# redwarp/kmeans-gpu

Hardware: AMD Instinct MI355X
Metric: pixels/sec per Lloyd iteration (8192x8192, k=256) (higher is better)
Workload: dtype f32; 1 GPU; synthetic uniform RGBA 8192x8192 (seed 0x5EED0003), k=256, one Lloyd iteration = update + assign (labels written every iteration) + accumulate; width=8192, height=8192, k=256, collective_backend=none (one rank), collective_ranks=1, label_pass=before the next iteration, update=by the last launch of the assign pass (kmg_lloyd_assign_update)

## Files before the change

### kmeans-gpu_amd/csrc/kmg_cube.hip

```cpp

#include "kmg_internal.h"
#include "kmg_table_dev.h"

#include <hip/hip_fp16.h>
#include <stdlib.h>

namespace kmg {

typedef float f32x2 __attribute__((ext_vector_type(2)));


namespace {

constexpr uint32_t kMaxListed = 32;
constexpr uint32_t kMaxLong = 256;
constexpr uint32_t kLongFlag = 0x200u;

__device__ __forceinline__ uint32_t sel3(uint32_t i, uint32_t x0, uint32_t x1, uint32_t x2)
{
    return i == 0u ? x0 : (i == 1u ? x1 : x2);
}

__device__ __forceinline__ int round_dir(int g, int m)
{
    const int a = g < 0 ? -g : g;
    const int r = (4 * a >= 3 * m ? 1 : 0) + (4 * a >= m ? 1 : 0);
    return g < 0 ? -r : r;
}

typedef unsigned short u16x2 __attribute__((ext_vector_type(2)));

__device__ __forceinline__ uint32_t group8_or(uint32_t v)
{
    v |= dpp_u32<kDppXor1>(v);
    v |= dpp_u32<kDppXor2>(v);
    v |= dpp_u32<kDppHalfMirror>(v);
    return v;
}

__device__ __forceinline__ uint32_t group8_min_u32(uint32_t v)
{
    v = min(v, dpp_u32<kDppXor1>(v));
    v = min(v, dpp_u32<kDppXor2>(v));
    v = min(v, dpp_u32<kDppHalfMirror>(v));
    return v;
}

__device__ __forceinline__ uint32_t group8_max_u32(uint32_t v)
{
    v = max(v, dpp_u32<kDppXor1>(v));
    v = max(v, dpp_u32<kDppXor2>(v));
    v = max(v, dpp_u32<kDppHalfMirror>(v));
    return v;
}



__device__ __forceinline__ uint32_t cell_pair_entry(const uint32_t idx[8], uint32_t occ, uint32_t lane)
{
    uint32_t rem = occ;
    uint32_t lab0 = 0, lab1 = 0, lab2 = 0, cnt0 = 0, cnt1 = 0, cnt2 = 0, msk0 = 0, msk1 = 0, msk2 = 0, n_occ = 0;
#pragma unroll
    for (int t = 0; t < 3; ++t) {
        const unsigned long long any = __ballot(rem != 0u);
        if (any) {
            uint32_t mine = 0;
#pragma unroll
            for (int q = 7; q >= 0; --q) mine = ((rem >> q) & 1u) ? idx[q] : mine;
            const uint32_t v = lane_value(mine, (uint32_t)__builtin_ctzll(any));
            uint32_t mm = 0;
#pragma unroll
            for (int q = 0; q < 8; ++q) mm |= (idx[q] == v ? 1u : 0u) << q;
            mm &= rem;
            rem &= ~mm;
            const uint32_t packed = wave_add_u32((uint32_t)__builtin_popcount(mm) | (t == 0 ? (uint32_t)__builtin_popcount(occ) << 10 : 0u));
            const uint32_t c = packed & 1023u;
            if (t == 0) { lab0 = v; msk0 = mm; cnt0 = c; n_occ = packed >> 10; }
            if (t == 1) { lab1 = v; msk1 = mm; cnt1 = c; }
            if (t == 2) { lab2 = v; msk2 = mm; cnt2 = c; }
        }
    }
    uint32_t a = 0;
    if (cnt1 > cnt0) a = 1;
    if (cnt2 > sel3(a, cnt0, cnt1, cnt2)) a = 2;
    uint32_t b = a == 0u ? 1u : 0u;
    if (a != 1u && b != 1u && cnt1 > sel3(b, cnt0, cnt1, cnt2)) b = 1;
    if (a != 2u && cnt2 > sel3(b, cnt0, cnt1, cnt2)) b = 2;
    const uint32_t labA = sel3(a, lab0, lab1, lab2), labB = sel3(b, lab0, lab1, lab2);
    const uint32_t mA = sel3(a, msk0, msk1, msk2), mB = sel3(b, msk0, msk1, msk2);
    const uint32_t rest = occ & ~mA;
    const uint32_t nA = sel3(a, cnt0, cnt1, cnt2), nR = n_occ - nA;
    if (nR == 0u) return pair_entry(labA, labA, 0u, 0u, 0u);

    const uint32_t half = ((lane >> 5) & 1u) | (((lane >> 4) & 1u) << 10) | (((lane >> 3) & 1u) << 20);
    const uint32_t hR = wave_add_u32((uint32_t)__builtin_popcount(rest) * half);
    const uint32_t hA = wave_add_u32((uint32_t)__builtin_popcount(mA) * half);
    const int gx = (int)((hR & 1023u) * nA) - (int)((hA & 1023u) * nR);
    const int gy = (int)(((hR >> 10) & 1023u) * nA) - (int)(((hA >> 10) & 1023u) * nR);
    const int gz = (int)((hR >> 20) * nA) - (int)((hA >> 20) * nR);
    const int ax = gx < 0 ? -gx : gx, ay = gy < 0 ? -gy : gy, az = gz < 0 ? -gz : gz;
    const int m = ax > ay ? (ax > az ? ax : az) : (ay > az ? ay : az);
    int nx = 2, ny = 0, nz = 0;
    if (m > 0) { nx = round_dir(gx, m); ny = round_dir(gy, m); nz = round_dir(gz, m); }

    const int xl = (int)(((lane >> 5) & 1u) * 4u + ((lane >> 1) & 3u));
    const int yl = (int)(((lane >> 4) & 1u) * 4u + (lane & 1u) * 2u);
    const int zl = (int)(((lane >> 3) & 1u) * 4u);
    const int bias = 7 * ((nx < 0 ? -nx : 0) + (ny < 0 ? -ny : 0) + (nz < 0 ? -nz : 0));
    const int p0 = nx * xl + ny * yl + nz * zl + bias;
    int p[8];
#pragma unroll
    for (int q = 0; q < 8; ++q) p[q] = p0 + ny * (q >> 2) + nz * (q & 3);
    const uint32_t notB = occ & ~mB;
    uint32_t tl = 63u, hi = 64u;
#pragma unroll
    for (int q = 0; q < 8; ++q) {
        if ((rest >> q) & 1u) tl = min(tl, (uint32_t)p[q]);
        if ((notB >> q) & 1u) hi = min(hi, (uint32_t)(63 - p[q]));
    }
    u16x2 packed = __builtin_bit_cast(u16x2, tl | (hi << 16));
    packed = __builtin_elementwise_min(packed, __builtin_bit_cast(u16x2, dpp_u32<kDppXor1>(__builtin_bit_cast(uint32_t, packed))));
    packed = __builtin_elementwise_min(packed, __builtin_bit_cast(u16x2, dpp_u32<kDppXor2>(__builtin_bit_cast(uint32_t, packed))));
    packed = __builtin_elementwise_min(packed, __builtin_bit_cast(u16x2, dpp_u32<kDppHalfMirror>(__builtin_bit_cast(uint32_t, packed))));
    packed = __builtin_elementwise_min(packed, __builtin_bit_cast(u16x2, dpp_u32<kDppMirror>(__builtin_bit_cast(uint32_t, packed))));
    packed = __builtin_elementwise_min(packed, __builtin_bit_cast(u16x2, (uint32_t)__builtin_amdgcn_update_dpp(-1, (int)__builtin_bit_cast(uint32_t, packed), 0x142, 0xA, 0xF, false)));
    packed = __builtin_elementwise_min(packed, __builtin_bit_cast(u16x2, (uint32_t)__builtin_amdgcn_update_dpp(-1, (int)__builtin_bit_cast(uint32_t, packed), 0x143, 0xC, 0xF, false)));
    const uint32_t pk = lane_value(__builtin_bit_cast(uint32_t, packed), 63);
    const int tlo = (int)(pk & 0xFFFFu);
    const int thi = 63 - (int)(pk >> 16);
    const int w = thi + 1 > tlo ? thi + 1 - tlo : 0;
    const uint32_t code = pair_dir_code(nx, ny, nz);
    if (w <= 6) return pair_entry(labA, labB, code, (uint32_t)tlo, (uint32_t)w);
    uint32_t low = 0, high = 0;
#pragma unroll
    for (int q = 0; q < 8; ++q) {
        if ((occ >> q) & 1u) { low += p[q] < tlo ? 1u : 0u; high += p[q] > thi ? 1u : 0u; }
    }
    const uint32_t lh = wave_add_u32(low | (high << 10));
    if ((lh & 1023u) >= (lh >> 10)) return pair_entry(labA, labB, code, (uint32_t)tlo, 7u);
    const int range = 7 * ((nx < 0 ? -nx : nx) + (ny < 0 ? -ny : ny) + (nz < 0 ? -nz : nz));
    return pair_entry(labB, labA, pair_dir_code(-nx, -ny, -nz), (uint32_t)(range - thi), 7u);
}

__device__ __forceinline__ uint32_t merge_state(uint32_t a, uint32_t b)
{
    return (a == kSubEmpty) ? b : ((b == kSubEmpty || b == a) ? a : (uint32_t)kSubMixed);
}

template <typename LabelT>
__device__ __forceinline__ void store_labels64(LabelT *dst64, uint32_t label, uint32_t lane)
{
    if (sizeof(LabelT) == 1) {
        const uint32_t t = label | (dpp_u32<kDppXor1>(label) << 8);
        const uint32_t u = t | (dpp_u32<kDppXor2>(t) << 16);
        if ((lane & 3u) == 0u) reinterpret_cast<uint32_t *>(dst64)[lane >> 2] = u;
    } else {
        const uint32_t t = label | (dpp_u32<kDppXor1>(label) << 16);
        if ((lane & 1u) == 0u) reinterpret_cast<uint32_t *>(dst64)[lane >> 1] = t;
    }
}


struct alignas(16) CellWork {
    uint16_t list[kMaxListed];
    unsigned long long br[4];
    uint32_t npop;
    uint32_t scan_set;
    uint32_t pad[6];
};
static_assert(sizeof(CellWork) == 128, "CellWork layout");

constexpr uint32_t kPairPending = 0xFFFFFFFEu;

constexpr uint32_t kLongSegs = 16, kLongSegCap = kCells / kLongSegs, kLongCount = 0, kLongCells = 64;
constexpr size_t kListsWords = kLongCells + kCells;
constexpr uint32_t kItemCands = 12;

__device__ __forceinline__ void flush_bins(const unsigned long long *bins, uint32_t k, uint32_t repl, uint32_t bin_stride,
                                           int64_t *sums, uint32_t n_rows)
{
    __syncthreads();
    unsigned long long *row = reinterpret_cast<unsigned long long *>(sums) + (uint64_t)(blockIdx.x % n_rows) * 4ull * k;
    for (uint32_t i = threadIdx.x; i < 4u * k; i += blockDim.x) {
        unsigned long long v = 0ull;
        for (uint32_t r = 0; r < repl; ++r) v += bins[(uint64_t)r * bin_stride + i];
        if (v) atomicAdd(row + i, v);
    }
}

__device__ __forceinline__ uint2 long_list_stage(const float4 *s_cent, const unsigned long long *s_masks, uint16_t *s_long,
                                              unsigned long long *s_sub, float4 sb0, float4 sb1, float4 sb2, uint32_t npop,
                                              uint32_t words, uint64_t *sub_masks_cell)
{
    const uint32_t lane = threadIdx.x & 63u;
// ... 1423 lines not shown
            } else if (valid) {
                uint4 *dst = reinterpret_cast<uint4 *>(s_lbl + slot * kCellColours + sub * 64u);
                dst[0] = xv; dst[1] = xv; dst[2] = xv; dst[3] = xv;
            }
        }
        unsigned long long pend0_b = 0ull;
        {
            const uint32_t rank = (uint32_t)__builtin_popcount(scan8 & ((1u << sub) - 1u));
            const bool head = open && (rank & 1u) == 0u;
            const uint32_t after = scan8 & ~((2u << sub) - 1u);
            const uint32_t s1 = after ? (uint32_t)__builtin_ctz(after) : 8u;
            const uint32_t un = listed ? (nm | ((head && s1 < 8u) ? s_mask[threadIdx.x - sub + s1] : 0u)) : 0u;
            const uint32_t n_un = (uint32_t)__builtin_popcount(un);
            const uint32_t type = unlisted ? 2u : (n_un > kItemCands ? 1u : 0u);
            const bool pend = valid && !uniform && sub == 0u;
            if (pend) s_left[slot] = ((uint32_t)__builtin_popcount(scan8) + 1u) >> 1;
            pend0_b = __ballot(pend && scan8 == 0u);
            const unsigned long long item_b = __ballot(head);
            if (bal_state) {
                const uint32_t cost = wave_add_u32(head ? 4u + (type == 2u ? npop : n_un) : 0u);
                if (lane == 0u) bal_state[(bal_pass & 1u) * 2u * kOneTaskSlots + kOneTaskSlots + blockIdx.x * kOneWaves + wv] = (uint16_t)min(cost, 65535u);
            }
            uint32_t i_base = 0u;
            if (lane == 0u && item_b) i_base = atomicAdd(&s_count[0], (uint32_t)__builtin_popcountll(item_b));
            i_base = __builtin_amdgcn_readfirstlane(i_base);
            if (head) {
                uint32_t iw0 = un, iw1 = 0u, iw2 = 0u;
                if (type == 0u) {
                    iw0 = 0u;
                    uint32_t q = 0u;
                    for (uint32_t m = un; m; m &= m - 1u, ++q) {
                        const uint32_t cc = (uint32_t)s_list[slot * kMaxListed + (uint32_t)__builtin_ctz(m)] << (8u * (q & 3u));
                        iw0 |= q < 4u ? cc : 0u; iw1 |= (q >= 4u && q < 8u) ? cc : 0u; iw2 |= q >= 8u ? cc : 0u;
                    }
                }
                s_item[i_base + bits_below_lane(item_b)] = make_uint4(slot | (sub << 7) | (s1 << 10) | (n_un << 14) | (type << 30), iw0, iw1, iw2);
            }
            if (stats) {
                st_single += (uint32_t)__builtin_popcountll(__ballot(single && sub == 0u));
                st_multi += (uint32_t)__builtin_popcountll(__ballot(valid && !single && sub == 0u));
                st_unlisted += (uint32_t)__builtin_popcountll(__ballot(unlisted && sub == 0u));
                st_decided += (uint32_t)__builtin_popcountll(__ballot(was_decided));
                st_scanned += (uint32_t)__builtin_popcountll(__ballot(mine || (unlisted && occupied)));
                st_cands += wave_add_u32(mine ? np0 : ((unlisted && occupied) ? npop : 0u));
                st_removed += wave_add_u32((uint32_t)__builtin_popcount(sm & ~nm));
                st_one += (uint32_t)__builtin_popcountll(__ballot(one));
            }
        }
        KMG_STAMP(4);
        __syncthreads();
        const uint32_t n_items = s_count[0];
        KMG_STAMP_VALUE(8, n_items); KMG_STAMP_VALUE(10, s_count[8]);

        auto cell_entry = [&](const uint32_t ps) {
            const uint32_t pcell = __builtin_amdgcn_readfirstlane(s_cell[ps]);
            const uint2 lv = *reinterpret_cast<const uint2 *>(s_lbl + ps * kCellColours + lane * 8u);
            uint32_t e = kPairPending;
            if (!(flags & kCubeNoEntries)) {
                const uint32_t occ = (uint32_t)s_occ[ps * 64u + lane];
                uint32_t idx[8];
#pragma unroll
                for (uint32_t q = 0; q < 4u; ++q) { idx[q] = (lv.x >> (8u * q)) & 0xFFu; idx[4u + q] = (lv.y >> (8u * q)) & 0xFFu; }
                e = cell_pair_entry(idx, occ, lane);
            }
            if (lane == 0u) pair_entries[pcell] = e;
            *reinterpret_cast<uint2 *>(colour_labels + (uint64_t)pcell * kCellColours + lane * 8u) = lv;
        };

        {
            uint32_t A_h = 0u, A_w0 = 0u, A_w1 = 0u, A_w2 = 0u, B_h = 0u, B_w0 = 0u, B_w1 = 0u, B_w2 = 0u, C_h = 0u, C_w0 = 0u, C_w1 = 0u, C_w2 = 0u;
            float4 A_v0, A_v1, B_v0, B_v1, C_v0, C_v1;
            uint32_t A_c0 = 1u, A_c1 = 1u, B_c0 = 1u, B_c1 = 1u, C_c0 = 1u, C_c1 = 1u;
            long long A_g = 0, B_g = 0, C_g = 0;
            bool A_ok = false, B_ok = false, C_ok = false;
#define KMG_REQUEST_ITEM(X)                                                                                       \
            do {                                                                                                  \
                uint32_t next_ = 0u;                                                                              \
                if (lane == 0u) next_ = atomicAdd(&s_count[4], 1u);                                               \
                next_ = __builtin_amdgcn_readfirstlane(next_);                                                    \
                X##_ok = next_ < n_items;                                                                         \
                const uint4 it_ = s_item[next_ < n_items ? next_ : 0u];                                           \
                X##_h = __builtin_amdgcn_readfirstlane(it_.x); X##_w0 = __builtin_amdgcn_readfirstlane(it_.y);    \
                X##_w1 = __builtin_amdgcn_readfirstlane(it_.z); X##_w2 = __builtin_amdgcn_readfirstlane(it_.w);   \
                const uint32_t cell_ = __builtin_amdgcn_readfirstlane(s_cell[X##_h & 127u]);                       \
                const uint32_t c0_ = cell_ * kCellColours + ((X##_h >> 7) & 7u) * 64u + lane;                     \
                const uint32_t c1_ = cell_ * kCellColours + ((X##_h >> 10) & 7u) * 64u + lane;    \
                X##_v0 = lab_table[c0_]; X##_v1 = lab_table[c1_];                                                 \
                if (SUMS) { X##_c0 = hist[c0_]; X##_c1 = hist[c1_]; X##_g = sub_agg[(uint64_t)cell_ * 32u + (lane & 31u)]; } \
            } while (0)
            auto scan_item = [&](const uint32_t hdr, const uint32_t w0, const uint32_t w1, const uint32_t w2, const float4 v0, const float4 v1,
                                 const uint32_t cnt0, const uint32_t cnt1, const long long sagg) {
                const uint32_t islot = hdr & 127u, s0 = (hdr >> 7) & 7u, s1 = (hdr >> 10) & 15u, n = (hdr >> 14) & 63u, type = hdr >> 30;
                const PixelTerms pt0 = pixel_terms_fast(v0.x, v0.y, v0.z, v0.w), pt1 = pixel_terms_fast(v1.x, v1.y, v1.z, v1.w);
                uint32_t ix0 = 0u, ix1 = 0u;
                if (type == 0u) {
                    const uint32_t my_cand = ((lane < 4u ? w0 : (lane < 8u ? w1 : w2)) >> (8u * (lane & 3u))) & 0xFFu;
                    uint32_t b0 = 0x7F7FFFFFu, r0 = 0x7F7FFFFFu, b1 = 0x7F7FFFFFu, r1 = 0x7F7FFFFFu;
                    const f32x2 qL = {pt0.L, pt1.L}, qa = {pt0.a, pt1.a}, qb = {pt0.b, pt1.b}, qC = {pt0.C, pt1.C};
                    const f32x2 qwC = {pt0.wC, pt1.wC}, qwH = {pt0.wH, pt1.wH};
                    auto cand_at = [&](uint32_t p) { return ((p < 4u ? w0 : (p < 8u ? w1 : w2)) >> (8u * (p & 3u))) & 0xFFu; };
                    for (uint32_t p = 0; p < n; ++p) {
                        const float4 c = s_cent[cand_at(p)];
                        const f32x2 dL = qL - c.x, da = qa - c.y, db = qb - c.z, dC = qC - c.w;
                        const f32x2 dC2 = dC * dC;
                        const f32x2 t = __builtin_elementwise_fma(db, db, da * da);
                        f32x2 h = t - dC2;
                        h.x = fmaxf(h.x, 0.0f); h.y = fmaxf(h.y, 0.0f);
// ... 278 lines not shown
```

### kmeans-gpu_amd/csrc/kmg_diffuse.hip

```cpp

#include "kmg_diffuse_dev.h"

namespace kmg {

namespace {

template <int ROUTE, bool ALPHA, typename OutT>
__global__ __launch_bounds__(64) void k_diffuse(const uint32_t *__restrict__ rgba, uint32_t w, uint32_t rows,
                                                OutT *__restrict__ out, uint2 *__restrict__ erow, uint32_t parity,
                                                DiffCtl *__restrict__ ctl, uint32_t *__restrict__ sticky, const Centroid *__restrict__ cent, uint32_t k,
                                                const float *__restrict__ lut, const uint32_t *__restrict__ pal,
                                                const void *__restrict__ colour_labels, const uint16_t *__restrict__ sub_table,
                                                uint32_t cutoff)
{
    constexpr uint32_t kLdsWords = ROUTE == kDiffusePairs ? kPairsLds : ROUTE == kDiffuseCells ? kCellsLds : 4u * 3072u + 256u + 3072u;
    __shared__ __attribute__((aligned(16))) uint32_t s_lds[kLdsWords];
    const uint32_t lane = threadIdx.x;
    float4 *s_cent = nullptr;
    float *s_lut = nullptr;
    uint32_t *s_pal;
    if (ROUTE == kDiffusePairs) {
        const uint4 *src = reinterpret_cast<const uint4 *>(sub_table + kSubCells + kCells);
        uint4 *dst = reinterpret_cast<uint4 *>(s_lds);
        for (uint32_t i = lane; i < kCells / 4; i += 64) dst[i] = src[i];
        for (uint32_t i = lane; i < 128; i += 64) s_lds[kCells + i] = i < kPairDirs ? pair_dir_word(i) : 0u;
        s_pal = s_lds + kCells + 128;
    } else if (ROUTE == kDiffuseCells) {
        const uint4 *src = reinterpret_cast<const uint4 *>(sub_table + kSubCells);
        uint4 *dst = reinterpret_cast<uint4 *>(s_lds);
        for (uint32_t i = lane; i < kCells / 8; i += 64) dst[i] = src[i];
        s_pal = s_lds + kCells / 2;
    } else {
        s_cent = reinterpret_cast<float4 *>(s_lds);
        for (uint32_t i = lane; i < k; i += 64) { const Centroid c = cent[i]; s_cent[i] = make_float4(c.L, c.a, c.b, c.C); }
        s_lut = reinterpret_cast<float *>(s_lds + 4u * 3072u);
        for (uint32_t i = lane; i < 256; i += 64) s_lut[i] = lut[i];
        s_pal = s_lds + 4u * 3072u + 256u;
    }
    for (uint32_t i = lane; i < k; i += 64) s_pal[i] = pal[i] | 0xFF000000u;
    __syncthreads();

    const uint32_t n_chunks = (rows + 63u) / 64u;
    for (;;) {
        uint32_t t = 0;
        if (lane == 0) t = __hip_atomic_fetch_add(&ctl->ticket, 1u, __ATOMIC_RELAXED, __HIP_MEMORY_SCOPE_AGENT);
        t = __builtin_amdgcn_readfirstlane(__shfl(t, 0));
        if (t >= n_chunks || timed_out(ctl)) return;
        const uint32_t y0 = t * 64u, nr = min(64u, rows - y0);
        const bool row_ok = lane < nr;
        const uint64_t row_base = (uint64_t)(y0 + (row_ok ? lane : 0u)) * w;
        const uint2 *e_in = erow + (size_t)((parity + t) & 1u) * w;
        uint2 *e_out = erow + (size_t)((parity + t + 1u) & 1u) * w;
        uint32_t known = t == 0 ? w : 0u;
        uint32_t published = 0;
        int eL[3] = {0, 0, 0}, am1[3] = {0, 0, 0}, a0[3] = {0, 0, 0}, ap1[3] = {0, 0, 0};
        uint2 eo = make_uint2(0u, 0u);
        const int steps = (int)w + 2 * ((int)nr - 1);
        bool abandoned = false;
        uint32_t beats = 0;
        heartbeat(ctl, t, beats);
        for (int s0 = 0; s0 < steps; s0 += kBody) {
            const uint32_t need = (uint32_t)min((long long)s0 + kBody + 1, (long long)w);
            if (known < need && !wait_progress(ctl, sticky, t, need, known, beats)) { abandoned = true; break; }
            heartbeat(ctl, t, beats);
            uint2 blk = make_uint2(0u, 0u);
            if (lane < (uint32_t)kBody && s0 + 1 + (int)lane < (int)w) blk = e_in[s0 + 1 + lane];
            if (s0 == 0 && lane == 0) {
                const uint2 z = e_in[0];
                ap1[0] = (int)(int16_t)(z.x & 0xFFFFu); ap1[1] = (int)z.x >> 16; ap1[2] = (int)z.y;
            }
            const int xb = s0 - 2 * (int)lane;
            uint32_t px[kBody];
#pragma unroll
            for (int j = 0; j < kBody; ++j) {
                const int x = xb + j;
                px[j] = (row_ok && x >= 0 && x < (int)w) ? rgba[row_base + (uint32_t)x] : 0u;
            }
            uint32_t ob[kBody];
// ... 107 lines not shown
```

### kmeans-gpu_amd/csrc/kmg_diffuse_wide.hip

```cpp

#include "kmg_diffuse_dev.h"
#include "kmg_diffusion.h"

namespace kmg {

namespace {

__device__ __forceinline__ void unpack_err(uint2 v, int e[3])
{
    e[0] = (int)(int16_t)(v.x & 0xFFFFu); e[1] = (int)v.x >> 16; e[2] = (int)v.y;
}

template <int ROUTE, bool ALPHA, typename OutT, int SKEW>
__global__ __launch_bounds__(64) void k_diffuse_wide(const uint32_t *__restrict__ rgba, uint32_t w, uint32_t rows,
                                                     OutT *__restrict__ out, uint2 *__restrict__ erow, uint32_t parity,
                                                     DiffCtl *__restrict__ ctl, uint32_t *__restrict__ sticky, const Centroid *__restrict__ cent, uint32_t k,
                                                     const float *__restrict__ lut, const uint32_t *__restrict__ pal,
                                                     const void *__restrict__ colour_labels, const uint16_t *__restrict__ sub_table,
                                                     uint32_t cutoff, const DiffuseFilter f)
{
    constexpr int R = SKEW - 1;
    constexpr uint32_t kLdsWords = ROUTE == kDiffusePairs ? kPairsLds : ROUTE == kDiffuseCells ? kCellsLds : 4u * 3072u + 256u + 3072u;
    __shared__ __attribute__((aligned(16))) uint32_t s_lds[kLdsWords];
    const uint32_t lane = threadIdx.x;
    float4 *s_cent = nullptr;
    float *s_lut = nullptr;
    uint32_t *s_pal;
    if (ROUTE == kDiffusePairs) {
        const uint4 *src = reinterpret_cast<const uint4 *>(sub_table + kSubCells + kCells);
        uint4 *dst = reinterpret_cast<uint4 *>(s_lds);
        for (uint32_t i = lane; i < kCells / 4; i += 64) dst[i] = src[i];
        for (uint32_t i = lane; i < 128; i += 64) s_lds[kCells + i] = i < kPairDirs ? pair_dir_word(i) : 0u;
        s_pal = s_lds + kCells + 128;
    } else if (ROUTE == kDiffuseCells) {
        const uint4 *src = reinterpret_cast<const uint4 *>(sub_table + kSubCells);
        uint4 *dst = reinterpret_cast<uint4 *>(s_lds);
        for (uint32_t i = lane; i < kCells / 8; i += 64) dst[i] = src[i];
        s_pal = s_lds + kCells / 2;
    } else {
        s_cent = reinterpret_cast<float4 *>(s_lds);
        for (uint32_t i = lane; i < k; i += 64) { const Centroid c = cent[i]; s_cent[i] = make_float4(c.L, c.a, c.b, c.C); }
        s_lut = reinterpret_cast<float *>(s_lds + 4u * 3072u);
        for (uint32_t i = lane; i < 256; i += 64) s_lut[i] = lut[i];
        s_pal = s_lds + 4u * 3072u + 256u;
    }
    for (uint32_t i = lane; i < k; i += 64) s_pal[i] = pal[i] | 0xFF000000u;
    __syncthreads();

    const uint32_t n_chunks = (rows + 63u) / 64u;
    for (;;) {
        uint32_t t = 0;
        if (lane == 0) t = __hip_atomic_fetch_add(&ctl->ticket, 1u, __ATOMIC_RELAXED, __HIP_MEMORY_SCOPE_AGENT);
        t = __builtin_amdgcn_readfirstlane(__shfl(t, 0));
        if (t >= n_chunks || timed_out(ctl)) return;
        const uint32_t y0 = t * 64u, nr = min(64u, rows - y0);
        const bool row_ok = lane < nr;
        const uint64_t row_base = (uint64_t)(y0 + (row_ok ? lane : 0u)) * w;
        const uint2 *e_in1 = erow + (size_t)((parity + t) & 1u) * 2u * w, *e_in2 = e_in1 + w;
        uint2 *e_out1 = erow + (size_t)((parity + t + 1u) & 1u) * 2u * w, *e_out2 = e_out1 + w;
        uint32_t known = t == 0 ? w : 0u;
        uint32_t published = 0;
        int eL1[3] = {0, 0, 0}, eL2[3] = {0, 0, 0};
        int u1[5][3], u2[5][3];
        uint2 pk[R + 1];
#pragma unroll
        for (int i = 0; i < 5; ++i)
#pragma unroll
            for (int c = 0; c < 3; ++c) u1[i][c] = u2[i][c] = 0;
#pragma unroll
        for (int q = 0; q <= R; ++q) pk[q] = make_uint2(0u, 0u);
        uint2 eo = make_uint2(0u, 0u);
        const int steps = (int)w + SKEW * ((int)nr - 1);
        bool abandoned = false;
        uint32_t beats = 0;
        heartbeat(ctl, t, beats);
        for (int s0 = 0; s0 < steps; s0 += kBody) {
            const uint32_t need = (uint32_t)min((long long)s0 + kBody + R, (long long)w);
            if (known < need && !wait_progress(ctl, sticky, t, need, known, beats)) { abandoned = true; break; }
            heartbeat(ctl, t, beats);
            uint2 blk1 = make_uint2(0u, 0u), blk2 = make_uint2(0u, 0u);
            const bool blk_ok = lane < (uint32_t)kBody && s0 + R + (int)lane < (int)w;
            if (blk_ok) { blk1 = e_in1[s0 + R + lane]; blk2 = e_in2[s0 + R + lane]; }
            if (nr == 1u && blk_ok) e_out2[s0 + R + lane] = blk1;
            if (s0 == 0) {
                uint2 p1 = make_uint2(0u, 0u), p2 = make_uint2(0u, 0u);
// ... 134 lines not shown
```

### kmeans-gpu_amd/csrc/kmg_index.hip

```cpp

#include "kmg_internal.h"
#include "kmg_table_dev.h"

namespace kmg {

namespace {

constexpr int kIndexBlock = 1024;

template <typename OutT, bool ALPHA, bool PAIRS>
__global__ __launch_bounds__(kIndexBlock) void k_labels_index(const uint32_t *__restrict__ rgba, uint64_t n,
                                                              const void *__restrict__ colour_labels,
                                                              const uint16_t *__restrict__ sub_table, uint32_t k,
                                                              OutT *__restrict__ out, int aligned, uint32_t cutoff)
{
    __shared__ uint32_t s_lds[PAIRS ? kCells + 128 : kCells / 2];
    if (PAIRS) {
        const uint4 *src = reinterpret_cast<const uint4 *>(sub_table + kSubCells + kCells);
        uint4 *dst = reinterpret_cast<uint4 *>(s_lds);
        for (uint32_t i = threadIdx.x; i < kCells / 4; i += kIndexBlock) dst[i] = src[i];
        if (threadIdx.x < 128) s_lds[kCells + threadIdx.x] = threadIdx.x < kPairDirs ? pair_dir_word(threadIdx.x) : 0u;
    } else {
        const uint4 *src = reinterpret_cast<const uint4 *>(sub_table + kSubCells);
        uint4 *dst = reinterpret_cast<uint4 *>(s_lds);
        for (uint32_t i = threadIdx.x; i < kCells / 8; i += kIndexBlock) dst[i] = src[i];
    }
    __syncthreads();
    const uint32_t *s_pair = s_lds, *s_dir = s_lds + kCells;
    const uint16_t *s_cell = reinterpret_cast<const uint16_t *>(s_lds);
    constexpr uint64_t TILE = (uint64_t)kIndexBlock * 8;
    const uint64_t tiles = (n + TILE - 1) / TILE;
    for (uint64_t tile = blockIdx.x; tile < tiles; tile += gridDim.x) {
        uint32_t px[8], ci[8];
        uint64_t i0[2];
#pragma unroll
        for (int g = 0; g < 2; ++g) {
            i0[g] = tile * TILE + (uint64_t)g * (kIndexBlock * 4) + (uint64_t)threadIdx.x * 4;
            load4_stream(rgba, i0[g], n, aligned != 0, px + g * 4);
#pragma unroll
            for (int q = 0; q < 4; ++q) ci[g * 4 + q] = colour_index(px[g * 4 + q]);
        }
        uint32_t lab[8];
        if (PAIRS) {
            bool fine[8];
#pragma unroll
            for (int p = 0; p < 8; ++p) {
                const uint32_t e = s_pair[ci[p] >> 9];
                const uint32_t dirw = s_dir[(e >> 16) & 127u];
                const uint32_t xyz = (px[p] & 0x00070707u) | 0x01000000u;
                const int proj = __builtin_amdgcn_sdot4((int)xyz, (int)dirw, 0, false);
                const int tlo = (int)((e >> 23) & 63u), w = (int)(e >> 29);
                const bool inA = proj < tlo, inB = proj >= tlo + w + (w == 7 ? 64 : 0);
                lab[p] = inA ? (e & 0xFFu) : ((e >> 8) & 0xFFu);
                fine[p] = !(inA || inB);
            }
#pragma unroll
            for (int p = 0; p < 8; ++p)
                if (fine[p]) lab[p] = (uint32_t)static_cast<const uint8_t *>(colour_labels)[ci[p]];
        } else {
#pragma unroll
            for (int p = 0; p < 8; ++p) lab[p] = (uint32_t)s_cell[ci[p] >> 9];
#pragma unroll
            for (int p = 0; p < 8; ++p)
                if (lab[p] == kSubMixed) lab[p] = (uint32_t)sub_table[ci[p] >> 6];
#pragma unroll
            for (int p = 0; p < 8; ++p)
                if (lab[p] == kSubMixed) lab[p] = (uint32_t)static_cast<const uint16_t *>(colour_labels)[ci[p]];
        }
#pragma unroll
        for (int p = 0; p < 8; ++p) lab[p] = index_of<ALPHA>(lab[p], px[p], cutoff, k);
#pragma unroll
        for (int g = 0; g < 2; ++g) store4_index<OutT, true>(out, i0[g], n, aligned != 0, lab + g * 4);
    }
}
// ... 49 lines not shown
```

### kmeans-gpu_amd/csrc/kmg_table.h

```cpp
#pragma once

#include <hip/hip_runtime.h>
#include <stdint.h>

#include "kmg_kernels.h"

namespace kmg {

constexpr uint32_t kCells = 32768;
constexpr uint32_t kCellColours = 512;
constexpr uint32_t kSubCells = kCells * 8;
constexpr uint32_t kCubeGrid = 2048;
constexpr uint32_t kMergeRows = 64;
constexpr uint32_t kHotMax = 56;
constexpr uint32_t kWorkWords = kCells + 1 + 1 + kHotMax;

constexpr uint16_t kSubEmpty = 0xFFFF;
constexpr uint16_t kSubMixed = 0xFFFE;

struct alignas(16) CellBounds {
    float L0, L1, a0, a1, b0, b1, C0, C1, wC0, wC1, wH0, wH1;
    float pad[4];
};

__host__ __device__ inline uint32_t colour_index(uint32_t px)
{
    const uint32_t cell = ((px << 16) & 0xF80000u) | ((px << 3) & 0x7C000u) | ((px >> 10) & 0x3E00u);
    const uint32_t low6 = (((px & 0x030303u) * 0x100401u) >> 16) & 63u;
    const uint32_t hi3 = (((px & 0x040404u) * 0x040201u) >> 12) & 0x1C0u;
    return cell | hi3 | low6;
}

__host__ __device__ inline uint32_t colour_index_reference(uint32_t px)
{
    const uint32_t r = px & 255u, g = (px >> 8) & 255u, b = (px >> 16) & 255u;
    return ((r >> 3) << 19) | ((g >> 3) << 14) | ((b >> 3) << 9) |
           (((r >> 2) & 1u) << 8) | (((g >> 2) & 1u) << 7) | (((b >> 2) & 1u) << 6) |
           ((r & 3u) << 4) | ((g & 3u) << 2) | (b & 3u);
}

__host__ __device__ inline void index_to_rgb(uint32_t idx, uint32_t &r, uint32_t &g, uint32_t &b)
{
    r = (((idx >> 19) & 31u) << 3) | (((idx >> 8) & 1u) << 2) | ((idx >> 4) & 3u);
    g = (((idx >> 14) & 31u) << 3) | (((idx >> 7) & 1u) << 2) | ((idx >> 2) & 3u);
    b = (((idx >> 9) & 31u) << 3) | (((idx >> 6) & 1u) << 2) | (idx & 3u);
}

inline uint32_t mask_words(uint32_t k) { return (k + 63u) / 64u; }
inline size_t cube_masks_bytes(uint32_t k)
{
    return sizeof(uint64_t) * ((size_t)kCells * mask_words(k) + (k <= 256 ? (size_t)kCells * 8u * 4u : 0u));
}

constexpr uint32_t kPairDirs = 125;
constexpr uint32_t kPairFine = 0xFFFFFFFFu;

__host__ __device__ inline uint32_t pair_dir_code(int nx, int ny, int nz)
{
    return (uint32_t)((nx + 2) * 25 + (ny + 2) * 5 + (nz + 2));
}

__host__ __device__ inline uint32_t pair_dir_word(uint32_t code)
{
    const int nx = (int)(code / 25u) - 2, ny = (int)((code / 5u) % 5u) - 2, nz = (int)(code % 5u) - 2;
    const int bias = 7 * ((nx < 0 ? -nx : 0) + (ny < 0 ? -ny : 0) + (nz < 0 ? -nz : 0));
    return ((uint32_t)nx & 255u) | (((uint32_t)ny & 255u) << 8) | (((uint32_t)nz & 255u) << 16) | ((uint32_t)bias << 24);
}

__host__ __device__ inline uint32_t pair_entry(uint32_t A, uint32_t B, uint32_t code, uint32_t tlo, uint32_t w)
{
    return (A & 255u) | ((B & 255u) << 8) | (code << 16) | (tlo << 23) | (w << 29);
}

__host__ __device__ inline int pair_project(uint32_t dir_word, uint32_t px)
{
    return (int)(int8_t)(dir_word & 255u) * (int)(px & 7u) + (int)(int8_t)((dir_word >> 8) & 255u) * (int)((px >> 8) & 7u) +
           (int)(int8_t)((dir_word >> 16) & 255u) * (int)((px >> 16) & 7u) + (int)(dir_word >> 24);
}

__host__ __device__ inline uint32_t pair_decode(uint32_t e, int p)
{
    const int tlo = (int)((e >> 23) & 63u);
    const int w = (int)(e >> 29);
    const int thr = tlo + w + (w == 7 ? 64 : 0);
    if (p < tlo) return e & 255u;
    if (p >= thr) return (e >> 8) & 255u;
    return kPairFine;
}

hipError_t launch_cell_bounds(const float *lut, CellBounds *bounds, CellBounds *sub_bounds, float4 *lab_table, hipStream_t st);
hipError_t launch_histogram(const uint32_t *rgba, uint64_t n, uint32_t *hist, hipStream_t st);
hipError_t launch_partitioned_histogram(const uint32_t *rgba, uint64_t n, uint64_t first_index, uint32_t *small,
                                        uint16_t *elems, uint32_t *keys, uint32_t *hist, uint32_t *tie, hipStream_t st);
hipError_t launch_cell_aggregates(const uint32_t *hist, const float4 *lab_table, int64_t *agg, int64_t *sub_agg, uint8_t *occ_bits,
                                  hipStream_t st);
hipError_t launch_work_list(const int64_t *agg, uint32_t *work, uint64_t n_pixels, hipStream_t st);
hipError_t launch_sparsity_probe(const uint32_t *rgba, uint64_t n, uint32_t *out3, hipStream_t st);
hipError_t launch_work_share(const uint32_t *work, uint32_t part, uint32_t parts, uint32_t *out, hipStream_t st);
hipError_t launch_tie_keys(const uint32_t *rgba, uint64_t n, uint64_t first_index, uint32_t *tie, hipStream_t st);
size_t init_scratch_bytes();
hipError_t launch_init_records(const uint32_t *work, const CellBounds *bounds, void *init_scratch, hipStream_t st);
hipError_t launch_init_pass_cells(const uint32_t *tie, const uint8_t *occ_bits, const float4 *lab_table, Centroid *cent,
                                  uint32_t j, int do_pass, float *dist, void *init_scratch, unsigned long long *band_key,
                                  const uint32_t *pick_rgba, const float *lut, hipStream_t st);
hipError_t launch_init_cells_multi(const uint32_t *tie, const uint8_t *occ_bits, const float4 *lab_table, Centroid *cent, uint32_t k,
                                   uint32_t launch, float *dist, void *init_scratch, const uint32_t *pick_rgba, const float *lut,
                                   hipStream_t st);
const uint32_t *init_cells_multi_count(const void *init_scratch, uint32_t launch);
size_t cube_work_bytes();
constexpr uint32_t kCubeNoEntries = 0x10000u;
constexpr uint32_t kCubeHot = 0x40000u;
constexpr uint32_t kCubeSplitLong = 0x80000u;
constexpr uint32_t kCubeSmallMaxK = 32;
bool cube_single_launch(uint32_t k, uint32_t flags);
hipError_t launch_cube_entries(const uint32_t *work, const uint8_t *occ_bits, const void *colour_labels, uint16_t *sub_table,
                               uint32_t k, hipStream_t st);
struct CubeTail {
    int64_t *acc_out = nullptr;
    int do_update = 0;
// ... 74 lines not shown
```

### kmeans-gpu_amd/csrc/kmg_table.hip

```cpp

#include "kmg_internal.h"
#include "kmg_table_dev.h"

#include <hip/hip_fp16.h>

namespace kmg {

__global__ __launch_bounds__(kBlock) void k_cell_bounds(const float *__restrict__ lut,
                                                        CellBounds *__restrict__ bounds,
                                                        CellBounds *__restrict__ sub_bounds,
                                                        float4 *__restrict__ lab_table)
{
    __shared__ float s_lut[256];
    __shared__ float s_min[6][8], s_max[6][8];
    s_lut[threadIdx.x] = lut[threadIdx.x];
    __syncthreads();
    const uint32_t wv = threadIdx.x >> 6, lane = threadIdx.x & 63;
#pragma unroll
    for (uint32_t pass = 0; pass < 2u; ++pass) {
        const uint32_t c = pass * kBlock + threadIdx.x;
        float L, a, b;
        colour_to_lab(s_lut, blockIdx.x * kCellColours + c, L, a, b);
        const PixelTerms p = pixel_terms(L, a, b);
        lab_table[blockIdx.x * kCellColours + c] = make_float4(p.L, p.a, p.b, p.C);
// ... 1198 lines not shown
        uint64_t i0[2];
#pragma unroll
        for (int g = 0; g < 2; ++g) {
            i0[g] = tile * TILE + (uint64_t)g * (kLabelBlock * 4) + (uint64_t)threadIdx.x * 4;
            uint32_t px[4];
            load4_stream(rgba, i0[g], n, aligned != 0, px);
#pragma unroll
            for (int q = 0; q < 4; ++q) ci[g * 4 + q] = colour_index(px[q]);
        }
        uint32_t lab[8];
#pragma unroll
        for (int p = 0; p < 8; ++p) lab[p] = (uint32_t)s_cell[ci[p] >> 9];
#pragma unroll
        for (int p = 0; p < 8; ++p)
            if (lab[p] == kSubMixed) lab[p] = (uint32_t)sub_table[ci[p] >> 6];
#pragma unroll
        for (int p = 0; p < 8; ++p)
            if (lab[p] == kSubMixed) lab[p] = (uint32_t)colour_labels[ci[p]];
        if (pal) {
#pragma unroll
            for (int p = 0; p < 8; ++p) lab[p] = s_pal[lab[p]];
        }
#pragma unroll
        for (int g = 0; g < 2; ++g) store4_stream(labels, i0[g], n, aligned != 0, lab + g * 4);
    }
}

constexpr uint32_t kHotCode = 127u;
constexpr size_t kLabelLdsPlain = sizeof(uint32_t) * (kCells + 256 + 128);
constexpr size_t kLabelLdsHot = kLabelLdsPlain + (size_t)kHotMax * kCellColours + sizeof(uint32_t) * 64;

template <bool HOT>
__global__ __launch_bounds__(kLabelBlock) void k_labels_pairs(const uint32_t *__restrict__ rgba, uint64_t n,
                                                              const uint8_t *__restrict__ colour_labels,
                                                              const uint32_t *__restrict__ pair_table,
                                                              const uint32_t *__restrict__ pal, uint32_t k,
                                                              uint32_t *__restrict__ labels, int aligned,
                                                              const uint32_t *__restrict__ hot, int64_t *__restrict__ tail_sums,
                                                              CubeTail tail)
{
    __shared__ uint32_t s_label_lds[(HOT ? kLabelLdsHot : kLabelLdsPlain) / sizeof(uint32_t)];
    if (tail.acc_out && blockIdx.x == gridDim.x - 1u) {
        for (uint32_t i = threadIdx.x; i < 4u * k; i += kLabelBlock) tail.acc_out[i] = tail_sums[i];
        if (tail.do_update) update_centroids(tail_sums, k, tail.convergence, tail.cent, tail.n_converged, s_label_lds, kLabelBlock);
        __syncthreads();
        for (uint32_t i = threadIdx.x; i < 4u * k; i += kLabelBlock) tail_sums[i] = 0;
        __syncthreads();
    }
    constexpr uint32_t kPairWords = kCells;
    uint32_t *s_pal = s_label_lds, *s_dir = s_label_lds + 256, *s_pair = s_label_lds + 256 + 128;
    uint8_t *s_hot = reinterpret_cast<uint8_t *>(s_label_lds + 256 + 128 + kPairWords);
    uint32_t *s_hcell = reinterpret_cast<uint32_t *>(s_hot + (size_t)kHotMax * kCellColours);
    if (pal && threadIdx.x < k) s_pal[threadIdx.x] = pal[threadIdx.x];
    if (threadIdx.x < 128) s_dir[threadIdx.x] = threadIdx.x < kPairDirs ? pair_dir_word(threadIdx.x) : 0u;
    {
        const uint4 *src = reinterpret_cast<const uint4 *>(pair_table);
        uint4 *dst = reinterpret_cast<uint4 *>(s_pair);
        for (uint32_t i = threadIdx.x; i < kPairWords / 4; i += kLabelBlock) dst[i] = src[i];
    }
    __syncthreads();
    if (HOT) {
        const uint32_t n_hot = min(hot[0], kHotMax);
        if (threadIdx.x < n_hot) {
            const uint32_t cell = hot[1u + threadIdx.x];
            const uint32_t e = s_pair[cell];
            const bool one_label = (e & 0xFFu) == ((e >> 8) & 0xFFu) && (e >> 23) == 0u;
            s_hcell[threadIdx.x] = one_label ? 0xFFFFFFFFu : cell;
        }
        __syncthreads();
        const uint32_t *lab32 = reinterpret_cast<const uint32_t *>(colour_labels);
        uint32_t *hot32 = reinterpret_cast<uint32_t *>(s_hot);
        for (uint32_t i = threadIdx.x; i < n_hot * (kCellColours / 4u); i += kLabelBlock) {
            const uint32_t cell = s_hcell[i / (kCellColours / 4u)];
            if (cell != 0xFFFFFFFFu) hot32[i] = lab32[(uint64_t)cell * (kCellColours / 4u) + (i % (kCellColours / 4u))];
        }
        if (threadIdx.x < n_hot && s_hcell[threadIdx.x] != 0xFFFFFFFFu)
            s_pair[s_hcell[threadIdx.x]] = threadIdx.x | (threadIdx.x << 8) | (kHotCode << 16);
        __syncthreads();
    }
    constexpr uint64_t TILE = (uint64_t)kLabelBlock * 8;
    const uint64_t tiles = (n + TILE - 1) / TILE;
    for (uint64_t tile = blockIdx.x; tile < tiles; tile += gridDim.x) {
        uint32_t ci[8], xyz[8];
        uint64_t i0[2];
#pragma unroll
        for (int g = 0; g < 2; ++g) {
            i0[g] = tile * TILE + (uint64_t)g * (kLabelBlock * 4) + (uint64_t)threadIdx.x * 4;
            uint32_t px[4];
            load4_stream(rgba, i0[g], n, aligned != 0, px);
#pragma unroll
            for (int q = 0; q < 4; ++q) {
                ci[g * 4 + q] = colour_index(px[q]);
                xyz[g * 4 + q] = (px[q] & 0x00070707u) | 0x01000000u;
            }
        }
        uint32_t lab[8];
        bool fine[8];
#pragma unroll
        for (int p = 0; p < 8; ++p) {
            const uint32_t e = s_pair[ci[p] >> 9];
            const uint32_t code = (e >> 16) & 127u;
            const uint32_t dirw = s_dir[code];
            const int proj = __builtin_amdgcn_sdot4((int)xyz[p], (int)dirw, 0, false);
            const int tlo = (int)((e >> 23) & 63u), w = (int)(e >> 29);
            const bool inA = proj < tlo, inB = proj >= tlo + w + (w == 7 ? 64 : 0);
            lab[p] = inA ? (e & 0xFFu) : ((e >> 8) & 0xFFu);
            fine[p] = !(inA || inB);
// ... 691 lines not shown
```

Before: 315.6 billion pixels/s.

## Refine pair-split directions with a quantized direction table and fused moment reductions

```diff
diff --git a/kmeans-gpu_amd/csrc/kmg_cube.hip b/kmeans-gpu_amd/csrc/kmg_cube.hip
--- a/kmeans-gpu_amd/csrc/kmg_cube.hip
+++ b/kmeans-gpu_amd/csrc/kmg_cube.hip
@@ -24,7 +24,7 @@
 __device__ __forceinline__ int round_dir(int g, int m)
 {
     const int a = g < 0 ? -g : g;
-    const int r = (4 * a >= 3 * m ? 1 : 0) + (4 * a >= m ? 1 : 0);
+    const int r = (6 * a >= m ? 1 : 0) + (2 * a >= m ? 1 : 0) + (6 * a >= 5 * m ? 1 : 0);
     return g < 0 ? -r : r;
 }
 
@@ -56,10 +56,64 @@
 
 
 
+__device__ __forceinline__ uint32_t xl_of(uint32_t lane) { return ((lane >> 5) & 1u) * 4u + ((lane >> 1) & 3u); }
+__device__ __forceinline__ uint32_t yl_of(uint32_t lane) { return ((lane >> 4) & 1u) * 4u + (lane & 1u) * 2u; }
+__device__ __forceinline__ uint32_t zl_of(uint32_t lane) { return ((lane >> 3) & 1u) * 4u; }
+__device__ __forceinline__ uint32_t lane_moment_z(uint32_t mask, uint32_t lane)
+{
+    return (uint32_t)__builtin_popcount(mask) * zl_of(lane) + (uint32_t)__builtin_popcount(mask & 0xAAu) +
+           2u * (uint32_t)__builtin_popcount(mask & 0xCCu);
+}
+
+struct PairSlab {
+    int tlo, thi, w;
+};
+
+__device__ __forceinline__ void pair_lane_p(uint32_t dirw, uint32_t lane, int p[8])
+{
+    const int nx = (int)(int8_t)(dirw & 255u), ny = (int)(int8_t)((dirw >> 8) & 255u), nz = (int)(int8_t)((dirw >> 16) & 255u);
+    const int p0 = nx * (int)xl_of(lane) + ny * (int)yl_of(lane) + nz * (int)zl_of(lane) + (int)(dirw >> 24);
+#pragma unroll
+    for (int q = 0; q < 8; ++q) p[q] = p0 + ny * (q >> 2) + nz * (q & 3);
+}
+
+__device__ __forceinline__ PairSlab pair_slab(const int p[8], uint32_t rest, uint32_t notB)
+{
+    uint32_t tl = 63u, hi = 64u;
+#pragma unroll
+    for (int q = 0; q < 8; ++q) {
+        if ((rest >> q) & 1u) tl = min(tl, (uint32_t)p[q]);
+        if ((notB >> q) & 1u) hi = min(hi, (uint32_t)(63 - p[q]));
+    }
+    u16x2 packed = __builtin_bit_cast(u16x2, tl | (hi << 16));
+    packed = __builtin_elementwise_min(packed, __builtin_bit_cast(u16x2, dpp_u32<kDppXor1>(__builtin_bit_cast(uint32_t, packed))));
+    packed = __builtin_elementwise_min(packed, __builtin_bit_cast(u16x2, dpp_u32<kDppXor2>(__builtin_bit_cast(uint32_t, packed))));
+    packed = __builtin_elementwise_min(packed, __builtin_bit_cast(u16x2, dpp_u32<kDppHalfMirror>(__builtin_bit_cast(uint32_t, packed))));
+    packed = __builtin_elementwise_min(packed, __builtin_bit_cast(u16x2, dpp_u32<kDppMirror>(__builtin_bit_cast(uint32_t, packed))));
+    packed = __builtin_elementwise_min(packed, __builtin_bit_cast(u16x2, (uint32_t)__builtin_amdgcn_update_dpp(-1, (int)__builtin_bit_cast(uint32_t, packed), 0x142, 0xA, 0xF, false)));
+    packed = __builtin_elementwise_min(packed, __builtin_bit_cast(u16x2, (uint32_t)__builtin_amdgcn_update_dpp(-1, (int)__builtin_bit_cast(uint32_t, packed), 0x143, 0xC, 0xF, false)));
+    const uint32_t pk = lane_value(__builtin_bit_cast(uint32_t, packed), 63);
+    PairSlab s;
+    s.tlo = (int)(pk & 0xFFFFu);
+    s.thi = 63 - (int)(pk >> 16);
+    s.w = s.thi + 1 > s.tlo ? s.thi + 1 - s.tlo : 0;
+    return s;
+}
+
+__device__ __forceinline__ uint32_t pair_sides(const int p[8], const PairSlab &s, uint32_t occ)
+{
+    uint32_t low = 0, high = 0;
+#pragma unroll
+    for (int q = 0; q < 8; ++q) {
+        if ((occ >> q) & 1u) { low += p[q] < s.tlo ? 1u : 0u; high += p[q] > s.thi ? 1u : 0u; }
+    }
+    return wave_add_u32(low | (high << 10));
+}
+
 __device__ __forceinline__ uint32_t cell_pair_entry(const uint32_t idx[8], uint32_t occ, uint32_t lane)
 {
     uint32_t rem = occ;
-    uint32_t lab0 = 0, lab1 = 0, lab2 = 0, cnt0 = 0, cnt1 = 0, cnt2 = 0, msk0 = 0, msk1 = 0, msk2 = 0, n_occ = 0;
+    uint32_t lab0 = 0, lab1 = 0, lab2 = 0, cnt0 = 0, cnt1 = 0, cnt2 = 0, msk0 = 0, msk1 = 0, msk2 = 0, n_occ = 0, sOx = 0, sOy = 0;
 #pragma unroll
     for (int t = 0; t < 3; ++t) {
         const unsigned long long any = __ballot(rem != 0u);
@@ -73,10 +127,13 @@
             for (int q = 0; q < 8; ++q) mm |= (idx[q] == v ? 1u : 0u) << q;
             mm &= rem;
             rem &= ~mm;
-            const uint32_t packed = wave_add_u32((uint32_t)__builtin_popcount(mm) | (t == 0 ? (uint32_t)__builtin_popcount(occ) << 10 : 0u));
+            const uint32_t c_occ = (uint32_t)__builtin_popcount(occ);
+            const uint32_t ride = t == 0 ? (c_occ << 10) | ((c_occ * xl_of(lane)) << 20)
+                                : t == 1 ? (c_occ * yl_of(lane) + (uint32_t)__builtin_popcount(occ & 0xF0u)) << 10 : 0u;
+            const uint32_t packed = wave_add_u32((uint32_t)__builtin_popcount(mm) | ride);
             const uint32_t c = packed & 1023u;
-            if (t == 0) { lab0 = v; msk0 = mm; cnt0 = c; n_occ = packed >> 10; }
-            if (t == 1) { lab1 = v; msk1 = mm; cnt1 = c; }
+            if (t == 0) { lab0 = v; msk0 = mm; cnt0 = c; n_occ = (packed >> 10) & 1023u; sOx = packed >> 20; }
+            if (t == 1) { lab1 = v; msk1 = mm; cnt1 = c; sOy = packed >> 10; }
             if (t == 2) { lab2 = v; msk2 = mm; cnt2 = c; }
         }
     }
@@ -92,54 +149,25 @@
     const uint32_t nA = sel3(a, cnt0, cnt1, cnt2), nR = n_occ - nA;
     if (nR == 0u) return pair_entry(labA, labA, 0u, 0u, 0u);
 
-    const uint32_t half = ((lane >> 5) & 1u) | (((lane >> 4) & 1u) << 10) | (((lane >> 3) & 1u) << 20);
-    const uint32_t hR = wave_add_u32((uint32_t)__builtin_popcount(rest) * half);
-    const uint32_t hA = wave_add_u32((uint32_t)__builtin_popcount(mA) * half);
-    const int gx = (int)((hR & 1023u) * nA) - (int)((hA & 1023u) * nR);
-    const int gy = (int)(((hR >> 10) & 1023u) * nA) - (int)(((hA >> 10) & 1023u) * nR);
-    const int gz = (int)((hR >> 20) * nA) - (int)((hA >> 20) * nR);
+    const uint32_t cA = (uint32_t)__builtin_popcount(mA);
+    const uint32_t mom1 = wave_add_u32((cA * xl_of(lane)) | ((cA * yl_of(lane) + (uint32_t)__builtin_popcount(mA & 0xF0u)) << 12));
+    const uint32_t mom2 = wave_add_u32(lane_moment_z(mA, lane) | (lane_moment_z(occ, lane) << 12));
+    const int gx = (int)(sOx * nA) - (int)((mom1 & 4095u) * n_occ);
+    const int gy = (int)(sOy * nA) - (int)(((mom1 >> 12) & 4095u) * n_occ);
+    const int gz = (int)(((mom2 >> 12) & 4095u) * nA) - (int)((mom2 & 4095u) * n_occ);
     const int ax = gx < 0 ? -gx : gx, ay = gy < 0 ? -gy : gy, az = gz < 0 ? -gz : gz;
     const int m = ax > ay ? (ax > az ? ax : az) : (ay > az ? ay : az);
-    int nx = 2, ny = 0, nz = 0;
-    if (m > 0) { nx = round_dir(gx, m); ny = round_dir(gy, m); nz = round_dir(gz, m); }
-
-    const int xl = (int)(((lane >> 5) & 1u) * 4u + ((lane >> 1) & 3u));
-    const int yl = (int)(((lane >> 4) & 1u) * 4u + (lane & 1u) * 2u);
-    const int zl = (int)(((lane >> 3) & 1u) * 4u);
-    const int bias = 7 * ((nx < 0 ? -nx : 0) + (ny < 0 ? -ny : 0) + (nz < 0 ? -nz : 0));
-    const int p0 = nx * xl + ny * yl + nz * zl + bias;
+    uint32_t code = pair_dir_code(3, 0, 0);
+    if (m > 0) code = pair_dir_code(round_dir(gx, m), round_dir(gy, m), round_dir(gz, m));
+
     int p[8];
-#pragma unroll
-    for (int q = 0; q < 8; ++q) p[q] = p0 + ny * (q >> 2) + nz * (q & 3);
-    const uint32_t notB = occ & ~mB;
-    uint32_t tl = 63u, hi = 64u;
-#pragma unroll
-    for (int q = 0; q < 8; ++q) {
-        if ((rest >> q) & 1u) tl = min(tl, (uint32_t)p[q]);
-        if ((notB >> q) & 1u) hi = min(hi, (uint32_t)(63 - p[q]));
-    }
-    u16x2 packed = __builtin_bit_cast(u16x2, tl | (hi << 16));
-    packed = __builtin_elementwise_min(packed, __builtin_bit_cast(u16x2, dpp_u32<kDppXor1>(__builtin_bit_cast(uint32_t, packed))));
-    packed = __builtin_elementwise_min(packed, __builtin_bit_cast(u16x2, dpp_u32<kDppXor2>(__builtin_bit_cast(uint32_t, packed))));
-    packed = __builtin_elementwise_min(packed, __builtin_bit_cast(u16x2, dpp_u32<kDppHalfMirror>(__builtin_bit_cast(uint32_t, packed))));
-    packed = __builtin_elementwise_min(packed, __builtin_bit_cast(u16x2, dpp_u32<kDppMirror>(__builtin_bit_cast(uint32_t, packed))));
-    packed = __builtin_elementwise_min(packed, __builtin_bit_cast(u16x2, (uint32_t)__builtin_amdgcn_update_dpp(-1, (int)__builtin_bit_cast(uint32_t, packed), 0x142, 0xA, 0xF, false)));
-    packed = __builtin_elementwise_min(packed, __builtin_bit_cast(u16x2, (uint32_t)__builtin_amdgcn_update_dpp(-1, (int)__builtin_bit_cast(uint32_t, packed), 0x143, 0xC, 0xF, false)));
-    const uint32_t pk = lane_value(__builtin_bit_cast(uint32_t, packed), 63);
-    const int tlo = (int)(pk & 0xFFFFu);
-    const int thi = 63 - (int)(pk >> 16);
-    const int w = thi + 1 > tlo ? thi + 1 - tlo : 0;
-    const uint32_t code = pair_dir_code(nx, ny, nz);
-    if (w <= 6) return pair_entry(labA, labB, code, (uint32_t)tlo, (uint32_t)w);
-    uint32_t low = 0, high = 0;
-#pragma unroll
-    for (int q = 0; q < 8; ++q) {
-        if ((occ >> q) & 1u) { low += p[q] < tlo ? 1u : 0u; high += p[q] > thi ? 1u : 0u; }
-    }
-    const uint32_t lh = wave_add_u32(low | (high << 10));
-    if ((lh & 1023u) >= (lh >> 10)) return pair_entry(labA, labB, code, (uint32_t)tlo, 7u);
-    const int range = 7 * ((nx < 0 ? -nx : nx) + (ny < 0 ? -ny : ny) + (nz < 0 ? -nz : nz));
-    return pair_entry(labB, labA, pair_dir_code(-nx, -ny, -nz), (uint32_t)(range - thi), 7u);
+    pair_lane_p(pair_dir_word(code), lane, p);
+    const PairSlab sl = pair_slab(p, rest, occ & ~mB);
+    if (sl.w <= 6) return pair_entry(labA, labB, code, (uint32_t)sl.tlo, (uint32_t)sl.w);
+    const uint32_t lh = pair_sides(p, sl, occ);
+    if ((lh & 1023u) >= (lh >> 10)) return pair_entry(labA, labB, code, (uint32_t)sl.tlo, 7u);
+    const uint32_t dirw = pair_dir_word(code);
+    return pair_entry(labB, labA, code ^ 1u, (dirw >> 24) + (pair_dir_word(code ^ 1u) >> 24) - (uint32_t)sl.thi, 7u);
 }
 
 __device__ __forceinline__ uint32_t merge_state(uint32_t a, uint32_t b)
@@ -1669,7 +1697,7 @@
         const uint32_t n_items = s_count[0];
         KMG_STAMP_VALUE(8, n_items); KMG_STAMP_VALUE(10, s_count[8]);
 
-        auto cell_entry = [&](const uint32_t ps) {
+        auto cell_entry = [&](const uint32_t ps) __attribute__((always_inline)) {
             const uint32_t pcell = __builtin_amdgcn_readfirstlane(s_cell[ps]);
             const uint2 lv = *reinterpret_cast<const uint2 *>(s_lbl + ps * kCellColours + lane * 8u);
             uint32_t e = kPairPending;
diff --git a/kmeans-gpu_amd/csrc/kmg_diffuse.hip b/kmeans-gpu_amd/csrc/kmg_diffuse.hip
--- a/kmeans-gpu_amd/csrc/kmg_diffuse.hip
+++ b/kmeans-gpu_amd/csrc/kmg_diffuse.hip
@@ -23,7 +23,7 @@
         const uint4 *src = reinterpret_cast<const uint4 *>(sub_table + kSubCells + kCells);
         uint4 *dst = reinterpret_cast<uint4 *>(s_lds);
         for (uint32_t i = lane; i < kCells / 4; i += 64) dst[i] = src[i];
-        for (uint32_t i = lane; i < 128; i += 64) s_lds[kCells + i] = i < kPairDirs ? pair_dir_word(i) : 0u;
+        for (uint32_t i = lane; i < 128; i += 64) s_lds[kCells + i] = pair_dir_word(i);
         s_pal = s_lds + kCells + 128;
     } else if (ROUTE == kDiffuseCells) {
         const uint4 *src = reinterpret_cast<const uint4 *>(sub_table + kSubCells);
diff --git a/kmeans-gpu_amd/csrc/kmg_diffuse_wide.hip b/kmeans-gpu_amd/csrc/kmg_diffuse_wide.hip
--- a/kmeans-gpu_amd/csrc/kmg_diffuse_wide.hip
+++ b/kmeans-gpu_amd/csrc/kmg_diffuse_wide.hip
@@ -30,7 +30,7 @@
         const uint4 *src = reinterpret_cast<const uint4 *>(sub_table + kSubCells + kCells);
         uint4 *dst = reinterpret_cast<uint4 *>(s_lds);
         for (uint32_t i = lane; i < kCells / 4; i += 64) dst[i] = src[i];
-        for (uint32_t i = lane; i < 128; i += 64) s_lds[kCells + i] = i < kPairDirs ? pair_dir_word(i) : 0u;
+        for (uint32_t i = lane; i < 128; i += 64) s_lds[kCells + i] = pair_dir_word(i);
         s_pal = s_lds + kCells + 128;
     } else if (ROUTE == kDiffuseCells) {
         const uint4 *src = reinterpret_cast<const uint4 *>(sub_table + kSubCells);
diff --git a/kmeans-gpu_amd/csrc/kmg_index.hip b/kmeans-gpu_amd/csrc/kmg_index.hip
--- a/kmeans-gpu_amd/csrc/kmg_index.hip
+++ b/kmeans-gpu_amd/csrc/kmg_index.hip
@@ -19,7 +19,7 @@
         const uint4 *src = reinterpret_cast<const uint4 *>(sub_table + kSubCells + kCells);
         uint4 *dst = reinterpret_cast<uint4 *>(s_lds);
         for (uint32_t i = threadIdx.x; i < kCells / 4; i += kIndexBlock) dst[i] = src[i];
-        if (threadIdx.x < 128) s_lds[kCells + threadIdx.x] = threadIdx.x < kPairDirs ? pair_dir_word(threadIdx.x) : 0u;
+        if (threadIdx.x < 128) s_lds[kCells + threadIdx.x] = pair_dir_word(threadIdx.x);
     } else {
         const uint4 *src = reinterpret_cast<const uint4 *>(sub_table + kSubCells);
         uint4 *dst = reinterpret_cast<uint4 *>(s_lds);
diff --git a/kmeans-gpu_amd/csrc/kmg_table.h b/kmeans-gpu_amd/csrc/kmg_table.h
--- a/kmeans-gpu_amd/csrc/kmg_table.h
+++ b/kmeans-gpu_amd/csrc/kmg_table.h
@@ -52,19 +52,68 @@
     return sizeof(uint64_t) * ((size_t)kCells * mask_words(k) + (k <= 256 ? (size_t)kCells * 8u * 4u : 0u));
 }
 
-constexpr uint32_t kPairDirs = 125;
+constexpr int8_t kPairExtra[][3] = {
+    {1, -3, 2}, {0, 3, -2}, {0, 3, -1}, {1, 3, -2}, {1, -3, 3}, {2, 1, -3}, {0, 2, -3},
+    {1, -3, 0}, {1, -2, 3}, {1, -3, 1}, {3, 1, -2}, {1, 3, -3}, {2, -3, 1}, {2, 3, -1},
+};
+constexpr uint32_t kPairDirs = 98u + 2u * (uint32_t)(sizeof(kPairExtra) / sizeof(kPairExtra[0]));
 constexpr uint32_t kPairFine = 0xFFFFFFFFu;
+static_assert(kPairDirs <= 127u, "code 127 is the hot-cell code");
+
+struct PairDirTable {
+    uint32_t word[128];
+    uint32_t near[343];
+};
+
+constexpr PairDirTable make_pair_dir_table()
+{
+    PairDirTable t = {};
+    int vec[64][3] = {};
+    int n_axes = 0;
+    for (int x = -2; x <= 0; ++x)
+        for (int y = -2; y <= 2; ++y)
+            for (int z = -2; z <= 2; ++z) {
+                const bool first_negative = x < 0 || (x == 0 && (y < 0 || (y == 0 && z < 0)));
+                const bool even = x % 2 == 0 && y % 2 == 0 && z % 2 == 0;
+                if (!first_negative || even) continue;
+                vec[n_axes][0] = -x; vec[n_axes][1] = -y; vec[n_axes][2] = -z;
+                ++n_axes;
+            }
+    for (unsigned i = 0; i < sizeof(kPairExtra) / sizeof(kPairExtra[0]); ++i, ++n_axes)
+        for (int c = 0; c < 3; ++c) vec[n_axes][c] = kPairExtra[i][c];
+    int norm2[64] = {};
+    for (int i = 0; i < n_axes; ++i) {
+        norm2[i] = vec[i][0] * vec[i][0] + vec[i][1] * vec[i][1] + vec[i][2] * vec[i][2];
+        for (int s = 0; s < 2; ++s) {
+            const int nx = s ? -vec[i][0] : vec[i][0], ny = s ? -vec[i][1] : vec[i][1], nz = s ? -vec[i][2] : vec[i][2];
+            const int bias = 7 * ((nx < 0 ? -nx : 0) + (ny < 0 ? -ny : 0) + (nz < 0 ? -nz : 0));
+            t.word[2 * i + s] = ((uint32_t)nx & 255u) | (((uint32_t)ny & 255u) << 8) | (((uint32_t)nz & 255u) << 16) | ((uint32_t)bias << 24);
+        }
+    }
+    for (int idx = 0; idx < 171; ++idx) {
+        const int qx = idx / 49 - 3, qy = idx / 7 % 7 - 3, qz = idx % 7 - 3;
+        int best = 0;
+        long long num = -1, den = 1;
+        for (int i = 0; i < n_axes; ++i) {
+            const int d = qx * vec[i][0] + qy * vec[i][1] + qz * vec[i][2];
+            if ((long long)d * d * den > num * norm2[i]) { best = 2 * i + (d < 0 ? 1 : 0); num = (long long)d * d; den = norm2[i]; }
+        }
+        t.near[idx] = (uint32_t)best;
+        t.near[342 - idx] = (uint32_t)best ^ 1u;
+    }
+    t.near[171] = 0u;
+    return t;
+}
+constexpr PairDirTable kPairDirTable = make_pair_dir_table();
 
 __host__ __device__ inline uint32_t pair_dir_code(int nx, int ny, int nz)
 {
-    return (uint32_t)((nx + 2) * 25 + (ny + 2) * 5 + (nz + 2));
+    return kPairDirTable.near[(nx + 3) * 49 + (ny + 3) * 7 + (nz + 3)];
 }
 
 __host__ __device__ inline uint32_t pair_dir_word(uint32_t code)
 {
-    const int nx = (int)(code / 25u) - 2, ny = (int)((code / 5u) % 5u) - 2, nz = (int)(code % 5u) - 2;
-    const int bias = 7 * ((nx < 0 ? -nx : 0) + (ny < 0 ? -ny : 0) + (nz < 0 ? -nz : 0));
-    return ((uint32_t)nx & 255u) | (((uint32_t)ny & 255u) << 8) | (((uint32_t)nz & 255u) << 16) | ((uint32_t)bias << 24);
+    return kPairDirTable.word[code & 127u];
 }
 
 __host__ __device__ inline uint32_t pair_entry(uint32_t A, uint32_t B, uint32_t code, uint32_t tlo, uint32_t w)
diff --git a/kmeans-gpu_amd/csrc/kmg_table.hip b/kmeans-gpu_amd/csrc/kmg_table.hip
--- a/kmeans-gpu_amd/csrc/kmg_table.hip
+++ b/kmeans-gpu_amd/csrc/kmg_table.hip
@@ -1274,7 +1274,7 @@
     uint8_t *s_hot = reinterpret_cast<uint8_t *>(s_label_lds + 256 + 128 + kPairWords);
     uint32_t *s_hcell = reinterpret_cast<uint32_t *>(s_hot + (size_t)kHotMax * kCellColours);
     if (pal && threadIdx.x < k) s_pal[threadIdx.x] = pal[threadIdx.x];
-    if (threadIdx.x < 128) s_dir[threadIdx.x] = threadIdx.x < kPairDirs ? pair_dir_word(threadIdx.x) : 0u;
+    if (threadIdx.x < 128) s_dir[threadIdx.x] = pair_dir_word(threadIdx.x);
     {
         const uint4 *src = reinterpret_cast<const uint4 *>(pair_table);
         uint4 *dst = reinterpret_cast<uint4 *>(s_pair);
```

Result: no change. 321.4 billion pixels/s, median of 6 (+1.9%).
